# kronbichler/multigrid

Measured on AMD Instinct MI355X. Metric: DoFs/s for Laplace matvec + V-cycle, poisson_cube p=4 fp64, higher is better.
Workload: dtype f64; 1 GPU; poisson_cube FE_Q(4) 128^3 cells, 135005697 DoFs per GPU, 8 levels, step = 1 fp64 vmult + 1 V-cycle (Chebyshev degree 3, first kind); cells_per_dim=128, degree=4, n_dofs_per_gpu=135005697, global_dofs=135005697, parallelism=1 GPU

## Files before the change

### multigrid_amd/csrc/mgx_api.cpp

```cpp
#include "../../include/mgx.h"
#include "mgx_bricks.hpp"
#include "mgx_device_memory.hpp"
#include "mgx_internal.hpp"

#include <hip/hip_runtime.h>
#include <rccl/rccl.h>

#include <dlfcn.h>

#include <algorithm>
#include <chrono>
#include <cmath>
#include <cstdio>
#include <cstdlib>
#include <cstring>
#include <memory>
#include <string>
#include <type_traits>
#include <utility>
#include <vector>

using namespace mgx;

namespace
// ... 28 lines not shown
#ifndef MGX_CELLS_FORM
#define MGX_CELLS_FORM 0
#endif
extern "C" int mgx_has_cells_form(void) { return MGX_CELLS_FORM; }
extern "C" int64_t mgx_live_device_allocations(void) { return mgx::live_device_allocations().load(); }

mgx::Tunables mgx::Tunables::from_environment()
{
  Tunables t;
  auto     num = [](const char *name, uint32_t dflt) {
    const char *e = std::getenv(name);
    return e ? (uint32_t)std::strtoul(e, nullptr, 10) : dflt;
  };
  t.trace               = std::getenv("MGX_TRACE") != nullptr;
  t.brick_min           = num("MGX_BRICK_MIN", t.brick_min);
  t.brick_min_from_env  = std::getenv("MGX_BRICK_MIN") != nullptr;
  t.overlap_min         = num("MGX_OVERLAP_MIN_BRICKS", t.overlap_min);
  t.restrict_colour_min = num("MGX_RESTRICT_COLOUR_MIN", t.restrict_colour_min);
  t.cell_colour_min     = num("MGX_CELL_COLOUR_MIN", t.cell_colour_min);
  t.free_max_bricks     = num("MGX_FREE_MAX_BRICKS", t.free_max_bricks);
  t.free_one_max        = num("MGX_FREE_ONE_MAX", t.free_one_max);
  t.graph_max_dofs      = num("MGX_GRAPH_MAX_DOFS", t.graph_max_dofs);
  return t;
}

bool mgx::Tunables::set(const std::string &name, double value)
{
  const bool     on = value != 0.;
  const uint32_t u  = value <= 0. ? 0u : (value >= 4294967295. ? 0xFFFFFFFFu : (uint32_t)value);
  struct Entry
  {
    const char *name;
    bool       *flag;
    uint32_t   *number;
  };
  const Entry table[] = {
    {"trace", &trace, nullptr},
    {"brick_min", nullptr, &brick_min},
    {"overlap_min_bricks", nullptr, &overlap_min},
    {"restrict_colour_min", nullptr, &restrict_colour_min},
    {"cell_colour_min", nullptr, &cell_colour_min},
    {"free_max_bricks", nullptr, &free_max_bricks},
    {"free_one_max", nullptr, &free_one_max},
    {"graph_max_dofs", nullptr, &graph_max_dofs},
    {"general_kernel", &general_kernel, nullptr},
    {"no_bricks", &no_bricks, nullptr},
#if MGX_CELLS_FORM
    {"cells_form", &cells_form, nullptr},
    {"brick_wide_max", nullptr, &wide_max},
#endif
    {"macro_wg_per_cu_x16", nullptr, &macro_wg_x16},
    {"no_diag_table", &no_diag_table, nullptr},
    {"no_macro_v2", &no_macro_v2, nullptr},
    {"no_general_bricks", &no_general_bricks, nullptr},
    {"general_brick_min", nullptr, &general_brick_min},
    {"fused_prolong_min_bricks", nullptr, &fused_prolong_min_bricks},
    {"roctx", &roctx, nullptr},
    {"no_fused_init", &no_fused_init, nullptr},
    {"no_fused_restrict", &no_fused_restrict, nullptr},
    {"no_fused_prolong", &no_fused_prolong, nullptr},
    {"force_fused_transfers", &force_fused_transfers, nullptr},
    {"transfer_v1", &transfer_v1, nullptr},
    {"restrict_atomic", &restrict_atomic, nullptr},
    {"exchange_unfused", &exchange_unfused, nullptr},
    {"no_graph", &no_graph, nullptr},
    {"dg_no_overlap", &dg_no_overlap, nullptr},
    {"dg_unmerged_restrict", &dg_unmerged_restrict, nullptr},
    {"no_fused_decomposed", &no_fused_decomposed, nullptr},
    {"no_fused_assembly", &no_fused_assembly, nullptr},
    {"no_fused_residual", &no_fused_residual, nullptr},
    {"no_restrict_scratch", &no_restrict_scratch, nullptr},
    {"rccl_selftest", &rccl_selftest, nullptr},
  };
  for (const Entry &e : table)
    if (name == e.name)
      {
        if (e.flag)
          *e.flag = on;
        else
          *e.number = u;
        if (name == "brick_min")
          brick_min_from_env = true;
        return true;
      }
  return false;
}

struct ExchangePlan
{
  std::vector<uint32_t> not_owned_host;
  int                    plan_id = 0, number = MGX_F64, self_pos = 0;
  std::vector<int>       rank;
  std::vector<uint32_t>  count;
  std::vector<uint32_t *> index_dev;
  std::vector<void *>    send, recv;
  uint32_t              *shared_dev = nullptr, *not_owned_dev = nullptr;
  uint32_t               n_shared = 0, n_not_owned = 0;
  void                  *own_buf = nullptr;
  std::vector<uint32_t>  start;
  uint32_t              *all_index_dev = nullptr, *csr_start_dev = nullptr, *csr_pos_dev = nullptr;
  uint8_t               *all_seg_dev = nullptr, *csr_k_dev = nullptr;
  bool                   fused = false;
};

struct RcclApi
{
// ... 1452 lines not shown
                    ck[fill[j]++] = 255;
                if (k < e.n_neighbors)
                  for (uint32_t i = 0; i < e.count[k]; ++i)
                    {
                      const uint32_t j = slot[e.index[k][i]];
                      ck[fill[j]]   = (uint8_t)k;
                      cp[fill[j]++] = i;
                    }
              }
            MGX_TRY(op.mem.upload(&P->all_index_dev, all_index));
            MGX_TRY(op.mem.upload(&P->all_seg_dev, all_seg));
            MGX_TRY(op.mem.upload(&P->csr_start_dev, cs));
            MGX_TRY(op.mem.upload(&P->csr_k_dev, ck));
            MGX_TRY(op.mem.upload(&P->csr_pos_dev, cp));
            P->fused = true;
          }
      }
    ctx->plans.push_back({(size_t)desc->n_dofs, P.get()});
    op.plan = std::move(P);
    return MGX_OK;
  }
}

extern "C" {

int mgx_operator_create(mgx_context_t ctx, const mgx_operator_desc *desc, mgx_operator_t *out)
{
  MGX_TRY(validate_operator_desc(ctx, desc, out));
  std::unique_ptr<mgx_operator_s, int (*)(mgx_operator_t)> op(new mgx_operator_s, mgx_operator_destroy);
  op->ctx              = ctx;
  op->constrained_last = constrained_are_last(desc);
  const Tunables &tun  = ctx->tun;
  const int       p = desc->degree, n = p + 1;
  const size_t    n_entries = 27 * (size_t)desc->n_cells;
  OperatorData   &d  = op->d;
  d.p              = p;
  d.number         = desc->number;
  d.n_cells        = desc->n_cells;
  d.n_dofs         = desc->n_dofs;
  d.n_constrained  = desc->n_constrained;
  for (int i = 0; i < 6; ++i)
    d.coef[i] = desc->coef[i];
  std::memcpy(op->S, desc->shape_values, sizeof(double) * n * n);
  std::memcpy(op->D, desc->colloc_grad, sizeof(double) * n * n);
  std::memcpy(op->w, desc->qweights, sizeof(double) * n);
  d.full_tensor      = !desc->coef_q && (desc->coef[3] != 0. || desc->coef[4] != 0. || desc->coef[5] != 0.);
  const bool general = d.full_tensor || desc->coef_q;
  d.separable        = !tun.general_kernel && !general;
  d.cells_form       = tun.cells_form;
  d.wide_max         = tun.wide_max;
  d.macro_wg_x16     = tun.macro_wg_x16;
  d.n_cus            = context_cus(ctx);
  d.macro_v2         = !tun.no_macro_v2;
  MGX_HIP(hipSetDevice(ctx->device));
  MGX_TRY(op->mem.upload(&d.idx27, desc->idx27, n_entries));
  if (desc->idx27_plain)
    MGX_TRY(op->mem.upload(&d.idx27_plain, desc->idx27_plain, n_entries));
  MGX_TRY(op->mem.upload(&d.constrained, desc->constrained, desc->n_constrained, 1));
  MGX_TRY(upload_basis(*op));
  MGX_TRY(op->mem.alloc(&d.inv_diag, number_size(d.number) * d.n_dofs));
  if (general)
    MGX_TRY(upload_general_tables(*op, desc));
  if (general && (desc->n_cells >= tun.cell_colour_min || (size_t)n * n * n * desc->n_cells > kAssemblyMaxEntries))
    MGX_TRY(colour_cells(*op, desc));
  const bool macro_covers = d.separable && (uint64_t)desc->n_dofs * number_size(d.number) < 0xFFFFFFF0ull;
  if (!tun.no_bricks && !general && (MGX_CELLS_FORM ? (p <= 4 || d.separable) : macro_covers))
    MGX_TRY(build_brick_schedule(*op, desc, tun));
  if (general && p == 4 && !desc->exchange && !tun.no_bricks && !tun.no_general_bricks && desc->n_dofs < 0x3FFFFFFFu &&
      (uint64_t)desc->n_dofs * number_size(d.number) < 0xFFFFFFF0ull &&
      desc->n_cells / 64 >= tun.general_brick_min)
    MGX_TRY(build_general_brick_schedule(*op, desc));
  MGX_TRY(build_ordered_assembly(*op, desc));
  start_vector_statistics(*op, desc);
  if (desc->global_index)
    MGX_TRY(op->mem.upload(&op->global_index_dev, desc->global_index, desc->n_dofs));
  if (desc->exchange)
    MGX_TRY(build_exchange_plan(*op, desc, tun));
  *out = op.release();
  return MGX_OK;
}

int mgx_operator_exchange_buffers(mgx_operator_t op, int k, void **send, void **recv, uint32_t *count, int *rank)
{
  MGX_REQUIRE(op && op->plan && k >= 0 && k < (int)op->plan->rank.size(), "mgx_operator_exchange_buffers: bad argument");
  if (send)
    *send = op->plan->send[k];
  if (recv)
    *recv = op->plan->recv[k];
  if (count)
    *count = op->plan->count[k];
  if (rank)
    *rank = op->plan->rank[k];
  return MGX_OK;
}

int mgx_exchange_add(mgx_operator_t op, void *vec)
{
  MGX_REQUIRE(op && vec, "mgx_exchange_add: null argument");
  return exchange_add(op, vec);
}

int mgx_operator_destroy(mgx_operator_t op)
{
  if (!op)
    return MGX_OK;
  (void)hipStreamSynchronize(op->ctx->stream);
// ... 2230 lines not shown
```

### multigrid_amd/csrc/mgx_internal.hpp

```cpp
#pragma once

#include "../../include/mgx.h"

#include <hip/hip_runtime.h>

#include <algorithm>
#include <cstddef>
#include <cstdint>
#include <string>
#include <type_traits>
#include <vector>

struct mgx_context_s;

namespace mgx
{
  constexpr int      kMaxN    = MGX_MAX_DEGREE + 1;
  constexpr uint32_t kInvalid = 0xFFFFFFFFu;

  struct Tunables
  {
    bool     trace            = false;
    bool     general_kernel   = false;
    bool     no_bricks        = false;
    uint32_t brick_min        = 512;
    bool     brick_min_from_env = false;
    uint32_t overlap_min      = 16384;
    bool     cells_form       = false;
    uint32_t wide_max         = 1024;
    bool     dg_no_overlap    = false;
    bool     no_restrict_scratch = false;
    bool     no_fused_residual = false;
    bool     no_fused_assembly = false;
    bool     no_fused_decomposed = false;
    bool     dg_unmerged_restrict = false;
    uint32_t macro_wg_x16     = 0;
    bool     no_diag_table    = false;
    bool     roctx            = false;
    uint32_t fused_prolong_min_bricks = 8192;
    bool     no_general_bricks = false;
    uint32_t general_brick_min = 2048;
    bool     no_macro_v2      = false;
    bool     no_fused_init    = false;
    bool     no_fused_restrict = false;
    bool     no_fused_prolong = false;
    bool     force_fused_transfers = false;
    bool     transfer_v1      = false;
    bool     restrict_atomic  = false;
    uint32_t restrict_colour_min = 16384;
    bool     exchange_unfused = false;
    uint32_t cell_colour_min  = 0xFFFFFFFFu;
    uint32_t free_max_bricks  = 16384;
    uint32_t free_one_max     = 1024;
    bool     no_graph         = false;
    uint32_t graph_max_dofs   = 600000;
    bool     rccl_selftest    = false;
    static Tunables from_environment();
    bool            set(const std::string &name, double value);
  };

  template <typename T>
  struct EOMat
  {
    T ee[(kMaxN / 2) * (kMaxN / 2)];
    T eo[(kMaxN / 2) * (kMaxN / 2)];
    T mc[kMaxN / 2];
    T mhh;
  };

  template <typename T>
  struct Basis1D
  {
    T S[kMaxN * kMaxN];
    T D[kMaxN * kMaxN];
    T w[kMaxN];
    T P1[2 * kMaxN * kMaxN];
    EOMat<T> mass, lapl;
    T P1eo[2 * kMaxN * kMaxN];
  };

  struct FreeSchedule
  {
    int       n_classes = 0;
    int       n_groups = 0, n_iface_groups = 0;
    uint32_t  group_start[9] = {0};
    uint32_t *ent         = nullptr;
    uint32_t *surf_off    = nullptr;
    uint32_t  n_surf      = 0;
    void     *priv        = nullptr;
    uint32_t *surf_dof    = nullptr, *surf_start = nullptr, *surf_pos = nullptr;
    uint32_t  n_surf_dofs = 0, n_surf_shared = 0;
    bool      available() const { return ent != nullptr; }
  };

  struct BrickData
  {
    uint32_t  n_bricks  = 0;
    int       n_colours = 0;
    int       n_iface_groups = 0;
    uint32_t  colour_start[33] = {0};
    uint32_t *ent_base  = nullptr;
    uint8_t  *ent_flags = nullptr;
    uint32_t *item_map  = nullptr;
    uint32_t *item_map2 = nullptr;
    std::vector<uint32_t> order;
    uint32_t *order_dev = nullptr;
    bool      available() const { return n_bricks > 0; }
    FreeSchedule fr;
  };
  constexpr int kBrickEntities = 729;
  constexpr int kMaxColours    = 32;

  struct OperatorData
  {
    int       p        = 0;
    int       number   = 1;
    uint32_t  n_cells  = 0;
    uint32_t  n_dofs   = 0;
    uint32_t  n_constrained = 0;
    uint32_t *idx27         = nullptr;
    uint32_t *idx27_plain   = nullptr;
    uint32_t *constrained   = nullptr;
    void     *basis         = nullptr;
    void     *inv_diag      = nullptr;
    double    coef[6]       = {0, 0, 0, 0, 0, 0};
    bool      full_tensor   = false;
    void     *coef_q        = nullptr;
    void     *grad_1d       = nullptr;
    uint32_t *cell_order    = nullptr;
    int       n_cell_colours = 0;
    uint32_t  cell_colour_start[33] = {0};
    uint32_t *asm_start     = nullptr;
    uint32_t *asm_pos       = nullptr;
    void     *cell_scratch  = nullptr;
    BrickData bricks;
    BrickData gbricks;
    bool      cells_form    = false;
    uint32_t  wide_max      = 1024;
    uint32_t  macro_wg_x16  = 0;
    uint32_t  n_cus         = 256;
    bool      separable     = true;
    void     *diag_items    = nullptr;
    void     *diag_items2   = nullptr;
    bool      macro_v2      = true;
  };

  struct TransferData
  {
    const OperatorData *coarse = nullptr, *fine = nullptr;
    uint32_t           *children = nullptr;
    uint8_t            *weight_shift = nullptr;
    uint32_t           *own27 = nullptr;
    uint32_t           *patch = nullptr;
    uint32_t           *coarse_blocks = nullptr;
    void               *coarse_scratch = nullptr;
    uint32_t           *cs_start = nullptr, *cs_pos = nullptr;
    uint32_t           *ifr_cdof = nullptr, *ifr_start = nullptr, *ifr_fdof = nullptr;
    void               *ifr_w = nullptr;
    uint32_t            n_ifr = 0;
    uint32_t           *ifp_start = nullptr, *ifp_cdof = nullptr;
    void               *ifp_w = nullptr;
    uint32_t            n_ifp = 0;
    mutable uint32_t    pipe_grid[4] = {0, 0, 0, 0};
    bool                owner_weights = false;
    bool                coarse_coloured = false;
    uint32_t            n_cus = 256;
    uint32_t            colour_min = 16384;
  };

  int  exchange_buffers(struct ::mgx_context_s *ctx, int plan_id, int number, int n_neighbors, const int *ranks,
                        const uint32_t *counts, void *const *send, void *const *recv, hipStream_t stream = nullptr);
  hipStream_t side_stream_begin(struct ::mgx_context_s *ctx);
  int         side_stream_end(struct ::mgx_context_s *ctx);
  int  allreduce_sum(struct ::mgx_context_s *ctx, double *values, int count);
  int  dot_owned_prefix(struct ::mgx_context_s *ctx, int number, const void *x, const void *y, size_t n, double *out);
  bool context_has_comm(struct ::mgx_context_s *ctx);
  const Tunables &context_tunables(struct ::mgx_context_s *ctx);
  void tridiag_extreme_eigenvalues(int n, const double *d, const double *e, double &lo, double &hi);

  int report_error(int code, const char *message);
  inline int report_error(int code, const std::string &message) { return report_error(code, message.c_str()); }

#define MGX_HIP(call)                                                                                                \
  do                                                                                                                 \
    {                                                                                                                \
      hipError_t e_ = (call);                                                                                        \
      if (e_ != hipSuccess)                                                                                          \
        return mgx::report_error(MGX_ERR_HIP, std::string(#call) + ": " + hipGetErrorString(e_) + " (" + __FILE__ + ":" + \
                                                std::to_string(__LINE__) + ")");                                     \
    }                                                                                                                \
  while (0)

#define MGX_TRY(call)     \
  do                      \
    {                     \
      int s_ = (call);    \
      if (s_ != MGX_OK)   \
// ... 323 lines not shown
```

### multigrid_amd/csrc/mgx_macro.hip

```cpp
#include "mgx_macro_device.hpp"

#include <hip/hip_runtime.h>

#include <algorithm>
#include <cstdlib>

#ifndef MGX_MACRO_CHUNK
#define MGX_MACRO_CHUNK (MGX_MACRO_PAIRS ? 3 : 4)
#endif
#ifndef MGX_MACRO_CHUNK_CHEB
#define MGX_MACRO_CHUNK_CHEB (MGX_MACRO_PAIRS ? 2 : 3)
#endif
#ifndef MGX_MACRO_T
#define MGX_MACRO_T double
#endif

#ifdef MGX_MACRO_STAMPS
#ifndef MGX_MACRO_STAMP_MODE
#define MGX_MACRO_STAMP_MODE -1
#endif
__device__ unsigned long long g_mgx_stamps[8192 * 16];
#define MGX_STAMP(k)                                                                    \
  do                                                                                    \
    {                                                                                   \
      if (threadIdx.x == 0 && blockIdx.x < 8192 && (MGX_MACRO_STAMP_MODE < 0 || MODE == MGX_MACRO_STAMP_MODE)) \
        g_mgx_stamps[blockIdx.x * 16 + (k)] = ((k) == 15 || (k) == 13) ? __builtin_amdgcn_s_memrealtime() \
                                                        : __builtin_amdgcn_s_memtime();  \
    }                                                                                   \
  while (0)
extern "C" int mgx_debug_read_stamps(unsigned long long *host, int n_blocks)
{
  return (int)hipMemcpyFromSymbol(host, HIP_SYMBOL(g_mgx_stamps), sizeof(unsigned long long) * 16 * n_blocks);
}
#define MGX_STAMP_IT(k)      \
  do                         \
    {                        \
      if (mgx_iter == 3)     \
        MGX_STAMP(k);        \
    }                        \
  while (0)
#define MGX_STAMP_NEXT() ++mgx_iter
#define mgx_iter_is(k) (mgx_iter == (k))
#else
#define MGX_STAMP(k) ((void)0)
#define MGX_STAMP_IT(k) ((void)0)
#define MGX_STAMP_NEXT() ((void)0)
#define mgx_iter_is(k) false
#endif

namespace mgx
{
  template <int P, typename T, int MODE, bool DTAB, bool FREE = false>
  __global__ void __launch_bounds__((MCfg<P, T>::THREADS), (MCfg<P, T>::MINW))
    brick_macro_kernel(const T *__restrict__ src, uint32_t brick_first, uint32_t brick_count,
                       const uint32_t *__restrict__ ent_base, const uint32_t *__restrict__ item_map,
                       const Basis1D<T> *__restrict__ B, T c0, T c1, T c2, BrickPost<T> post, uint32_t vec_bytes)
  {
    using C              = MCfg<P, T>;
    constexpr int G      = C::G;
    constexpr int NT     = C::THREADS;
    constexpr int IT     = C::IT;
    constexpr int LINES  = C::LINES;
    constexpr int NEW    = (C::NE + NT - 1) / NT;
    constexpr int N = P + 1, NB = C::NB;
    constexpr int REM    = LINES - NT;
    constexpr bool kKeepX = is_cheb_mode(MODE) || MODE == kCgUpdate;
    constexpr int  NG     = ((MODE == kChebInit && !DTAB) || MODE == kCgUpdate) ? 2 : 1;
    __shared__ T U[C::ASZ];
    __shared__ T W[C::ASZ];

    const int tid = threadIdx.x;
    uint32_t  b   = blockIdx.x;
    if (b >= brick_count)
      return;
    MGX_STAMP(0);
    MGX_STAMP(15);
#ifdef MGX_MACRO_STAGGER
    if (__builtin_amdgcn_s_getreg(6 | (0 << 6) | ((8 - 1) << 11)) != 0)
      for (int i = 0; i < MGX_MACRO_STAGGER; ++i)
        __builtin_amdgcn_s_sleep(64);
#endif
    constexpr int NP = C::NPAIR, NS = C::NSINGLE, JP = C::JP, JS = C::JS, NU = JP + JS;
    auto live_p = [&](int j) { return (j + 1) * NT <= NP || tid + j * NT < NP; };
    auto live_s = [&](int j) { return (j + 1) * NT <= NS || tid + j * NT < NS; };
    auto live   = [&](int v) { return v < 2 * JP ? live_p(v / 2) : live_s(v - 2 * JP); };
    uint32_t mw[IT];
#pragma unroll
    for (int j = 0; j < JP; ++j)
      {
        const int     q = tid + j * NT;
        const u32x2_t m = reinterpret_cast<const u32x2_t *>(item_map)[q < NP ? q : 0];
        mw[2 * j]       = m.x;
        mw[2 * j + 1]   = m.y;
      }
#pragma unroll
    for (int j = 0; j < JS; ++j)
      {
        const int q    = tid + j * NT;
        mw[2 * JP + j] = item_map[2 * NP + (q < NS ? q : 0)];
      }
    T dv[DTAB ? IT : 1];
    if (DTAB)
      {
#pragma unroll
        for (int j = 0; j < JP; ++j)
// ... 41 lines not shown
#pragma unroll
      for (int j = 0; j < NEW; ++j)
        if (tid + j * NT < C::NE)
          E[tid + j * NT] = e[j];
    };
    auto unit_offset = [&](uint32_t w, uint32_t m, int it = 0, uint32_t brick = 0) {
#ifdef MGX_MACRO_CONTIG
      return w != kInvalid ? ((brick_first + brick) * (uint32_t)(C::NB * C::NB * C::NB * P * P * P) + (uint32_t)(tid + it * NT)) * (uint32_t)sizeof(T) : kOob;
#else
      return w != kInvalid ? (ent_index(w) + item_offset(m)) * (uint32_t)sizeof(T) : kOob;
#endif
    };
    constexpr bool kProlong = MODE == kChebFirstProlong;
    constexpr int  CNP = (C::NB / 2) * P + 1, NCV = CNP * CNP * CNP / NT + 1, CE3 = (C::NB + 1) * (C::NB + 1) * (C::NB + 1);
    T              cvv[NCV];
    T    g[NG][IT];
    uint32_t cw[NCV];
    auto coarse_words = [&](uint32_t brick) {
      if (kProlong)
        {
          const uint32_t *ctab = post.coarse_blocks + (size_t)(brick_first + brick) * CE3;
#pragma unroll
          for (int k = 0; k < NCV; ++k)
            {
              const int l = tid + k * NT;
              int       slot = 0, pnt;
              uint32_t  off;
              if (l < CNP * CNP * CNP)
                coarse_point<P>(l, slot, off, pnt);
              cw[k] = ctab[slot];
            }
        }
    };
    auto coarse_values = [&]() {
      if (kProlong)
        {
#pragma unroll
          for (int k = 0; k < NCV; ++k)
            {
              const int l = tid + k * NT;
              cvv[k]      = T(0);
              if (l < CNP * CNP * CNP)
                {
                  int      slot, pnt;
                  uint32_t off;
                  coarse_point<P>(l, slot, off, pnt);
                  const uint32_t w = cw[k];
                  const T        v = post.coarse[w != kInvalid ? w + off : 0u];
                  cvv[k]           = w != kInvalid ? v : T(0);
                }
            }
        }
    };
    auto gather_issue = [&](const uint32_t *E, uint32_t brick) {
      const rsrc_t r0 = MODE == kChebInit ? (DTAB ? R.a : R.b) : rsrc;
      const rsrc_t r1 = MODE == kCgUpdate ? R.b : R.a;
#pragma unroll
      for (int j = 0; j < JP; ++j)
        {
#pragma unroll
          for (int e = 0; e < 2; ++e)
            g[0][2 * j + e] = g[NG - 1][2 * j + e] = T(0);
          if (live_p(j))
            {
              const uint32_t off = unit_offset(E[item_slot(mw[2 * j])], mw[2 * j], 2 * j, brick);
              buf_ld2(r0, off, g[0][2 * j], g[0][2 * j + 1]);
              if (NG == 2)
                buf_ld2(r1, off, g[NG - 1][2 * j], g[NG - 1][2 * j + 1]);
            }
        }
#pragma unroll
      for (int j = 0; j < JS; ++j)
        {
          const int v = 2 * JP + j;
          g[0][v] = g[NG - 1][v] = T(0);
          if (live_s(j))
            {
              const uint32_t off = unit_offset(E[item_slot(mw[v])], mw[v], v, brick);
              g[0][v]            = buf_ld(r0, off, T());
              if (NG == 2)
                g[NG - 1][v] = buf_ld(r1, off, T());
            }
        }
    };
    T    xs[kKeepX ? IT : 1];
    auto gather_land = [&]() {
#pragma unroll
      for (int it = 0; it < IT; ++it)
        {
          T v = g[0][it];
          if (MODE == kChebInit)
            v = DTAB ? post.f0 * dv[DTAB ? it : 0] * g[0][it] : post.f0 * g[0][it] * g[NG - 1][it];
          if (MODE == kCgUpdate)
            v = post.f1 == T(0) ? g[NG - 1][it] : post.f2 * g[0][it] + g[NG - 1][it];
          if (live(it))
            U[item_point(mw[it])] = v;
          if (kKeepX)
            xs[it] = v;
        }
    };

    auto interpolate = [&]() {
      if (kProlong)
        {
          lds_barrier();
          prolong_brick<P, T, NT>(tid, W, B->P1eo, cvv);
        }
    };
    auto add_correction = [&]() {
      if (kProlong)
        {
#pragma unroll
          for (int it = 0; it < IT; ++it)
            if (live(it))
              {
                const uint32_t pnt = item_point(mw[it]);
                xs[kKeepX ? it : 0] += W[pnt];
                U[pnt] = xs[kKeepX ? it : 0];
              }
        }
    };

    table_load(b, ec);
    table_store(reinterpret_cast<uint32_t *>(W), ec);
    __syncthreads();
    MGX_STAMP(1);
    gather_issue(reinterpret_cast<const uint32_t *>(W), b);
    coarse_words(b);
    coarse_values();
    interpolate();
    gather_land();
// ... 137 lines not shown
            for (int i = 0; i < N; ++i)
              seg[i] = W[base + i * (G * G)];
            cell_apply<P, T>(K, seg, r);
#pragma unroll
            for (int i = 0; i < N; ++i)
              seg[i] = U[base + i * (G * G)];
            cell_apply<P, T>(M, seg, y);
#pragma unroll
            for (int i = 0; i < N; ++i)
              y[i] = fma(c2, r[i], y[i]);
            const T yn = next_lane(y[0]);
            if (c + 1 < NB)
              y[P] += yn;
#pragma unroll
            for (int i = 1; i < N; ++i)
              W[base + i * (G * G)] = y[i];
            if (c == 0)
              W[base] = y[0];
          }
        if (tid < LINES)
          {
            const int l = tid;
            T         a[G], r[G], o[G];
#pragma unroll
            for (int j = 0; j < G; ++j)
              a[j] = W[l + j * (G * G)];
            macro_apply<P, T>(K, a, r);
#pragma unroll
            for (int j = 0; j < G; ++j)
              a[j] = U[l + j * (G * G)];
            macro_apply<P, T>(M, a, o);
#pragma unroll
            for (int j = 0; j < G; ++j)
              W[l + j * (G * G)] = fma(c2, r[j], o[j]);
          }
          }
#endif
        __syncthreads();
        MGX_STAMP_IT(6);
        uint32_t *ebase = reinterpret_cast<uint32_t *>(U), *E2 = ebase + C::NE;
        table_store(ebase, ec);
        if (has_next)
          table_store(E2, en);
        const uint32_t *sbase = ebase + 2 * C::NE;
        if (FREE)
          {
#pragma unroll
            for (int j = 0; j < NEW; ++j)
              if (tid + j * NT < C::NE)
                ebase[2 * C::NE + tid + j * NT] = sc[FREE ? j : 0];
          }
        __syncthreads();
        constexpr bool kPipeGather = (MODE != kChebInit || DTAB) && MODE != kCgUpdate && MODE != kChebFirstProlong;
        if (has_next && kPipeGather)
          gather_issue(E2, bn);
        if (has_next)
          coarse_values();
        MGX_STAMP_IT(7);

        {
          constexpr int kChunk = MODE == kPlain ? NU : (MODE == kResidual ? (NU + 1) / 2 : (kKeepX ? MGX_MACRO_CHUNK_CHEB : MGX_MACRO_CHUNK)),
                        NCH    = (NU + kChunk - 1) / kChunk;
          PostOps<T>    ops[2][kChunk];
          uint32_t      iw[2][kChunk];
          uint32_t      pw[2][FREE ? kChunk : 1];
          const uint32_t priv0 = FREE ? (brick_first + b) * post.n_surf : 0u;
          auto slot0 = [&](int u) { return u < JP ? 2 * u : JP + u; };
          auto ulive = [&](int u) { return u < JP ? live_p(u) : live_s(u - JP); };
          auto issue = [&](int c, PostOps<T>(&o)[kChunk], uint32_t(&w)[kChunk], uint32_t(&pv)[FREE ? kChunk : 1]) {
#pragma unroll
            for (int j = 0; j < kChunk; ++j)
              {
                const int u = c * kChunk + j;
                w[j]        = kInvalid;
                if (u < NU && ulive(u))
                  w[j] = ebase[item_slot(mw[slot0(u)])];
                if (FREE)
                  {
                    const uint32_t so = (u < NU && ulive(u)) ? sbase[item_slot(mw[slot0(u < NU ? u : 0)])] : kInvalid;
                    const bool     vd = w[j] != kInvalid;
                    if (vd && so != kInvalid)
                      w[j] = ent_index(w[j]) | 0x40000000u;
                    pv[FREE ? j : 0] = (vd && so != kInvalid)
                                         ? (priv0 + so + item_offset(mw[slot0(u < NU ? u : 0)])) * (uint32_t)sizeof(T)
                                         : kOob;
                  }
              }
#pragma unroll
            for (int j = 0; j < kChunk; ++j)
              {
                const int u = c * kChunk + j;
                if (u < JP)
                  post_issue<T, MODE, DTAB, true>(R, w[j], unit_offset(w[j], mw[slot0(u < NU ? u : 0)], slot0(u < NU ? u : 0), b), o[j]);
                else if (u < NU)
                  post_issue<T, MODE, DTAB, false>(R, w[j], unit_offset(w[j], mw[slot0(u < NU ? u : 0)], slot0(u < NU ? u : 0), b), o[j]);
              }
          };
          issue(0, ops[0], iw[0], pw[0]);
#pragma unroll
          for (int c = 0; c < NCH; ++c)
            {
              if (c + 1 < NCH)
                issue(c + 1, ops[(c + 1) & 1], iw[(c + 1) & 1], pw[(c + 1) & 1]);
              __builtin_amdgcn_sched_barrier(0);
              T val[kChunk][2];
#pragma unroll
              for (int j = 0; j < kChunk; ++j)
                {
                  const int u = c * kChunk + j;
                  val[j][0] = val[j][1] = T(0);
                  if (u < NU && ulive(u))
                    {
                      val[j][0] = W[item_point(mw[slot0(u)])];
                      if (u < JP)
                        val[j][1] = W[item_point(mw[slot0(u) + 1])];
                    }
                }
#pragma unroll
              for (int j = 0; j < kChunk; ++j)
                {
                  const int u = c * kChunk + j;
                  if (u < NU)
                    {
                      const int         v0   = slot0(u);
                      const bool        pair = u < JP;
                      const uint32_t    w    = iw[c & 1][j];
                      const bool        vld  = w != kInvalid, last = vld && (w >> 31);
                      const uint32_t    off  = unit_offset(w, mw[v0], v0, b);
                      const PostOps<T> &o    = ops[c & 1][j];
                      T                 res[2];
#pragma unroll
                      for (int e = 0; e < 2; ++e)
                        res[e] = (e == 0 || pair)
                                   ? post_finish<T, MODE>(post, o.pv[e], o.av[e], o.ov[e], DTAB ? dv[DTAB ? v0 + e : 0] : o.bv[e],
                                                          last, val[j][e], xs[kKeepX ? v0 + e : 0])
                                   : T(0);
                      constexpr int kStAux = (MODE == kPlain || MODE == kResidual) ? kAuxNt : 0;
                      auto          st     = [&](rsrc_t r, uint32_t f) {
                        if (pair)
                          buf_st2(r, f, res[0], res[1]);
                        else
                          buf_st<kStAux>(r, f, res[0]);
                      };
                      if (MODE == kResidualRestrict)
                        {
                          if (ulive(u))
                            {
                              W[item_point(mw[v0])] = vld ? res[0] : T(0);
                              if (pair)
                                W[item_point(mw[v0 + 1])] = vld ? res[1] : T(0);
                            }
                        }
                      else if (MODE == kCgUpdate)
                        {
                          st(R.out, last ? off : kOob);
                          if (__builtin_amdgcn_ballot_w64(vld && !last) != 0)
                            st(R.partial, last ? kOob : off);
                          const T xn = o.ov[0] + post.f1 * o.bv[0];
                          buf_st(R.srcw, last ? off : kOob, xs[kKeepX ? v0 : 0]);
                          if (post.f1 != T(0))
                            buf_st(R.xw, last ? off : kOob, xn);
                          if (last)
                            {
                              const double qv = (double)res[0], pn = (double)xs[kKeepX ? v0 : 0], rv = (double)o.av[0];
                              cg[0] += qv * pn;
                              cg[1] += rv * rv;
                              cg[2] += qv * rv;
                              cg[3] += qv * qv;
                            }
                        }
                      else
                        {
                          st(R.out, last ? off : kOob);
                          if (FREE)
                            {
                              const uint32_t po = pw[c & 1][FREE ? j : 0];
                              if (__builtin_amdgcn_ballot_w64(po != kOob) != 0)
                                st(R.priv, po);
                              if (__builtin_amdgcn_ballot_w64(vld && !last && po == kOob) != 0)
                                st(R.partial, (last || po != kOob) ? kOob : off);
                            }
#ifndef MGX_MACRO_NOCARRIER
                          else if (__builtin_amdgcn_ballot_w64(vld && !last) != 0)
                            st(R.partial, last ? kOob : off);
#endif
                          if (MODE == kChebFirstProlong)
                            buf_st(R.srcw, last ? off : kOob, xs[kKeepX ? v0 : 0]);
                        }
                    }
                }
              __builtin_amdgcn_sched_barrier(0);
            }
        }
        MGX_STAMP_IT(8);
        if (MODE == kResidualRestrict)
          {
            constexpr int CE1 = C::NB + 1;
            __syncthreads();
            const uint32_t *ctab = post.coarse_blocks + (size_t)(brick_first + b) * (CE1 * CE1 * CE1);
            if (post.coarse_scratch)
              restrict_brick<P, T, NT, true>(tid, W, B->P1eo, nullptr, ctab,
                                             post.coarse_scratch + (size_t)(brick_first + b) * (CNP * CNP * CNP));
            else
              restrict_brick<P, T, NT, false>(tid, W, B->P1eo, post.coarse, ctab);
          }
        if (!has_next)
          break;
        if (!kPipeGather)
          gather_issue(E2, bn);
        __syncthreads();
#pragma unroll
        for (int j = 0; j < NEW; ++j)
          ec[j] = en[j];
        interpolate();
        gather_land();
        add_correction();
        MGX_STAMP_IT(9);
        __syncthreads();
        MGX_STAMP_IT(10);
        b = bn;
        MGX_STAMP_NEXT();
      }
    if (MODE == kCgUpdate)
      {
        static_assert(MODE != kCgUpdate || !MGX_MACRO_PAIRS, "kCgUpdate is written for single items");
        __syncthreads();
        double *red = reinterpret_cast<double *>(U);
#pragma unroll
        for (int k = 0; k < 4; ++k)
          red[k * NT + tid] = cg[k];
        __syncthreads();
        constexpr int P2 = NT <= 64 ? 64 : (NT <= 128 ? 128 : (NT <= 256 ? 256 : 512));
        for (int stride = P2 / 2; stride > 0; stride >>= 1)
          {
            if (tid < stride && tid + stride < NT)
              {
#pragma unroll
                for (int k = 0; k < 4; ++k)
                  red[k * NT + tid] += red[k * NT + tid + stride];
              }
            __syncthreads();
          }
        if (tid < 4)
          post.sums[blockIdx.x * 4 + tid] = red[tid * NT];
      }
#ifdef MGX_MACRO_STAMPS
    asm volatile("s_waitcnt vmcnt(0)" ::: "memory");
    MGX_STAMP(14);
    MGX_STAMP(13);
#endif
  }

  template <int P, typename T, int MODE, bool FREE>
  static void macro_launch(hipStream_t s, const OperatorData &op, const T *src, BrickPost<T> post, int g0, int g1)
  {
    using C                     = MCfg<P, T>;
    const BrickData &bd         = op.bricks;
    const uint32_t  *ent        = FREE ? bd.fr.ent : bd.ent_base;
    const uint32_t  *group_start = FREE ? bd.fr.group_start : bd.colour_start;
    if (FREE)
      {
        post.priv       = (T *)bd.fr.priv;
        post.surf_off   = bd.fr.surf_off;
        post.n_surf     = bd.fr.n_surf;
        post.priv_bytes = (uint32_t)((size_t)bd.n_bricks * bd.fr.n_surf * sizeof(T));
      }
    constexpr bool kUsesDiag = is_cheb_mode(MODE);
    const bool     dtab      = kUsesDiag && op.diag_items;
    if (dtab)
      post.b = (const T *)op.diag_items;
    const bool one_launch = MODE == kResidualRestrict && post.coarse_scratch != nullptr;
    for (int c = g0; c < g1; ++c)
      {
        uint32_t first = group_start[c], count = group_start[c + 1] - first;
        if (one_launch)
          {
            if (c != g0)
              break;
            count = group_start[g1] - first;
          }
        if (count == 0)
          continue;
        const uint32_t grid = persistent_grid(op, C::WGS, count);
        if (dtab)
          hipLaunchKernelGGL((brick_macro_kernel<P, T, MODE, kUsesDiag, FREE>), dim3(grid), dim3(C::THREADS), 0, s, src, first,
                             count, ent, bd.item_map, (const Basis1D<T> *)op.basis, (T)op.coef[0], (T)op.coef[1],
                             (T)op.coef[2], post, (uint32_t)(op.n_dofs * sizeof(T)));
        else
          hipLaunchKernelGGL((brick_macro_kernel<P, T, MODE, false, FREE>), dim3(grid), dim3(C::THREADS), 0, s, src, first,
                             count, ent, bd.item_map, (const Basis1D<T> *)op.basis, (T)op.coef[0], (T)op.coef[1],
                             (T)op.coef[2], post, (uint32_t)(op.n_dofs * sizeof(T)));
      }
  }

#if MGX_MACRO_IS_F64
  __global__ void reduce4_kernel(const double *__restrict__ partials, uint32_t n, const double *__restrict__ extra,
                                 double *__restrict__ sums)
  {
    __shared__ double red[4 * 256];
    const int         tid = threadIdx.x;
    double            acc[4] = {0., 0., 0., 0.};
    for (uint32_t i = tid; i < n; i += 256)
      for (int k = 0; k < 4; ++k)
        acc[k] += partials[4 * (size_t)i + k];
    for (int k = 0; k < 4; ++k)
      red[k * 256 + tid] = acc[k];
    __syncthreads();
    for (int stride = 128; stride > 0; stride >>= 1)
      {
        if (tid < stride)
          for (int k = 0; k < 4; ++k)
            red[k * 256 + tid] += red[k * 256 + tid + stride];
        __syncthreads();
      }
    if (tid < 4)
      sums[tid] = red[tid * 256] + (extra ? extra[tid] : 0.);
  }
#endif

  template <typename T, bool VERIFY>
  __global__ void diag_table_kernel(const T *__restrict__ inv_diag, const uint32_t *__restrict__ ent_base,
                                    const uint32_t *__restrict__ item_map, uint32_t ne, uint32_t npts, T *table,
                                    uint32_t *flag)
  {
    const uint32_t brick = blockIdx.x;
    for (uint32_t i = threadIdx.x; i < npts; i += blockDim.x)
      {
        const uint32_t m = item_map[i], w = ent_base[(size_t)brick * ne + item_slot(m)];
        if (w == kInvalid)
          continue;
        const T v = inv_diag[ent_index(w) + item_offset(m)];
        if (!VERIFY)
          table[i] = v;
        else
          {
            const T    t   = table[i];
            const T    tol = (sizeof(T) == 8 ? T(1e-14) : T(2e-6)) * (t < 0 ? -t : t);
            const T    dvt = v - t;
            const bool same = (dvt < 0 ? -dvt : dvt) <= tol;
            if (!same)
              atomicOr(flag, 1u);
          }
      }
  }
// ... 101 lines not shown
```

### multigrid_amd/csrc/mgx_macro2.hip

```cpp
#include "mgx_macro_device.hpp"

#include <hip/hip_runtime.h>

#include <algorithm>
#include <cstdlib>

#ifndef MGX_MACRO_T
#define MGX_MACRO_T double
#endif
#ifndef MGX_MACRO2_CHUNK
#define MGX_MACRO2_CHUNK 3
#endif

#ifdef MGX_MACRO_STAMPS
#ifndef MGX_MACRO_STAMP_MODE
#define MGX_MACRO_STAMP_MODE -1
#endif
__device__ unsigned long long g_mgx_stamps2[8192 * 16];
#define MGX_STAMP(k)                                                                                              \
  do                                                                                                              \
    {                                                                                                             \
      if (threadIdx.x == 0 && blockIdx.x < 8192 && (MGX_MACRO_STAMP_MODE < 0 || MODE == MGX_MACRO_STAMP_MODE))      \
        g_mgx_stamps2[blockIdx.x * 16 + (k)] = ((k) == 15 || (k) == 13) ? __builtin_amdgcn_s_memrealtime()         \
                                                                         : __builtin_amdgcn_s_memtime();           \
// ... 146 lines not shown
#pragma unroll
        for (int j = 0; j < G; ++j)
          U[base + j * G] = fma(c0, t2[j], c1 * s2[j]);
      }
    lds_barrier();
    mark(1);
    if (REM > 0 && tid < REM * NB)
      {
        const int l = NT + tid / NB, c = tid % NB, base = l + c * P * (G * G);
        T         seg[N], y[N], r[N];
#pragma unroll
        for (int i = 0; i < N; ++i)
          seg[i] = W[base + i * (G * G)];
        cell_apply<P, T>(K, seg, r);
#pragma unroll
        for (int i = 0; i < N; ++i)
          seg[i] = U[base + i * (G * G)];
        cell_apply<P, T>(M, seg, y);
#pragma unroll
        for (int i = 0; i < N; ++i)
          y[i] = fma(c2, r[i], y[i]);
        const T yn = next_lane(y[0]);
        if (c + 1 < NB)
          y[P] += yn;
#pragma unroll
        for (int i = 1; i < N; ++i)
          W[base + i * (G * G)] = y[i];
        if (c == 0)
          W[base] = y[0];
      }
    if (tid < LINES)
      {
        const int l = tid;
        T         a[G], r[G], o[G];
#pragma unroll
        for (int j = 0; j < G; ++j)
          a[j] = W[l + j * (G * G)];
        macro_apply<P, T>(K, a, r);
#pragma unroll
        for (int j = 0; j < G; ++j)
          a[j] = U[l + j * (G * G)];
        macro_apply<P, T>(M, a, o);
#pragma unroll
        for (int j = 0; j < G; ++j)
          W[l + j * (G * G)] = fma(c2, r[j], o[j]);
      }
  }

  __host__ __device__ constexpr bool macro2_covers(int mode, int p)
  {
    return mode == kPlain || mode == kResidual || ((mode == kResidualRestrict || mode == kChebInit) && p <= 4) || mode == kChebOldInit;
  }

  template <int P, typename T, int MODE>
  __global__ void __launch_bounds__((M2Cfg<P, T>::THREADS), (M2Cfg<P, T>::MINW))
    brick_macro2_kernel(const T *__restrict__ src, uint32_t brick_first, uint32_t brick_count,
                        const uint32_t *__restrict__ ent_base, const uint32_t *__restrict__ item_map,
                        const Basis1D<T> *__restrict__ B, T c0, T c1, T c2, BrickPost<T> post, uint32_t vec_bytes)
  {
    static_assert(macro2_covers(MODE, P), "form not covered by this pipeline");
    using C            = M2Cfg<P, T>;
    constexpr int NT   = C::THREADS, IT = C::IT, JINT = C::JINT, JSURF = C::JSURF, NE = C::NE;
    constexpr int NEW  = (NE + NT - 1) / NT;
    __shared__ T        U[C::ASZ];
    __shared__ T        W[C::ASZ];
    __shared__ uint32_t E[NE];

    const int tid = threadIdx.x;
    uint32_t  b   = blockIdx.x;
    if (b >= brick_count)
      return;
    MGX_STAMP(0);
    MGX_STAMP(15);
#ifdef MGX_MACRO_STAMPS
    int mgx_iter = 0;
#endif
    auto live = [&](int j) { return (j + 1) * NT <= C::NPTS || tid + j * NT < C::NPTS; };
    uint32_t mw[IT];
#pragma unroll
    for (int j = 0; j < IT; ++j)
      mw[j] = item_map[live(j) ? tid + j * NT : 0];
    const rsrc_t rsrc = make_rsrc(src, vec_bytes), r_a = make_rsrc(post.a, vec_bytes), r_out = make_rsrc(post.out, vec_bytes),
                 r_partial = make_rsrc(post.partial, vec_bytes), r_old = make_rsrc(post.old, vec_bytes);
    const EOMat<T> &M = B->mass, &K = B->lapl;
    constexpr bool kKeepX = is_cheb_mode(MODE);
    T              dv[kKeepX ? IT : 1];
    if (kKeepX)
      {
#pragma unroll
        for (int j = 0; j < IT; ++j)
          dv[kKeepX ? j : 0] = post.b[live(j) ? tid + j * NT : 0];
      }

    uint32_t en[NEW] = {};
    auto     table_load = [&](uint32_t brick, uint32_t(&e)[NEW]) {
#pragma unroll
      for (int j = 0; j < NEW; ++j)
        {
          const int i = tid + j * NT;
          e[j]        = ent_base[(size_t)(brick_first + brick) * NE + (i < NE ? i : 0)];
        }
    };
    auto table_store = [&](uint32_t *dst, const uint32_t(&e)[NEW]) {
#pragma unroll
      for (int j = 0; j < NEW; ++j)
        if (tid + j * NT < NE)
          dst[tid + j * NT] = e[j];
    };
    auto unit_offset = [&](uint32_t w, uint32_t m) {
      return w != kInvalid ? (ent_index(w) + item_offset(m)) * (uint32_t)sizeof(T) : kOob;
    };
    T    g[IT];
    auto gather_issue = [&](const uint32_t *tab) {
#pragma unroll
      for (int j = 0; j < IT; ++j)
        {
          g[j] = T(0);
          if (live(j))
            g[j] = buf_ld(MODE == kChebInit ? r_a : rsrc, unit_offset(tab[item_slot(mw[j])], mw[j]), T());
        }
    };
    T    xs[kKeepX ? IT : 1];
    auto gather_land = [&]() {
#pragma unroll
      for (int j = 0; j < IT; ++j)
        {
          T v = g[j];
          if (MODE == kChebInit)
            v = post.f0 * dv[kKeepX ? j : 0] * g[j];
          if (live(j))
            U[item_point(mw[j])] = v;
          if (kKeepX)
            xs[kKeepX ? j : 0] = v;
        }
    };
    constexpr bool kCarrier = MODE != kResidualRestrict;
    T              pp[JSURF];
    auto           partial_issue = [&]() {
#pragma unroll
      for (int j = JINT; j < IT; ++j)
        {
          pp[j - JINT] = T(0);
          if (!kCarrier)
            continue;
#ifndef MGX_MACRO_NOCARRIER
          const uint32_t w    = live(j) ? E[item_slot(mw[j])] : kInvalid;
          const bool     need = w != kInvalid && !(w & 0x40000000u);
          if (__builtin_amdgcn_ballot_w64(need) != 0)
            pp[j - JINT] = buf_ld(r_partial, need ? unit_offset(w, mw[j]) : kOob, T());
#endif
        }
    };

    constexpr bool kRhs = MODE == kResidual || MODE == kResidualRestrict;
    T              av[kRhs ? IT : 1];
    auto           rhs_issue = [&]() {
      if (kRhs)
        {
#pragma unroll
          for (int j = 0; j < IT; ++j)
            {
              const uint32_t w    = live(j) ? E[item_slot(mw[j])] : kInvalid;
              const bool     last = w != kInvalid && (j < JINT || (w >> 31));
              av[kRhs ? j : 0]    = buf_ld(r_a, last ? unit_offset(w, mw[j]) : kOob, T());
            }
        }
    };

    {
      uint32_t e0[NEW];
      table_load(b, e0);
      if (b + gridDim.x < brick_count)
        table_load(b + gridDim.x, en);
      table_store(E, e0);
      lds_barrier();
      MGX_STAMP(1);
      gather_issue(E);
      gather_land();
      MGX_STAMP(2);
      lds_barrier();
    }

    for (;;)
      {
        const uint32_t bn = b + gridDim.x;
        const bool     has_next = bn < brick_count;
        MGX_STAMP_IT(3);
#ifdef MGX_MACRO_STAMPS
        if (mgx_iter == 4)
          MGX_STAMP(11);
#endif
        partial_issue();
        rhs_issue();
#pragma unroll
        for (int j = 0; j < IT; ++j)
          asm volatile("" : "+v"(mw[j]));
        if (MODE == kChebInit || MODE == kChebOldInit)
          {
#pragma unroll
            for (int j = 0; j < IT; ++j)
              asm volatile("" : "+v"(dv[kKeepX ? j : 0]));
          }
        MGX_STAMP_IT(4);
#ifndef MGX_MACRO_NOSWEEP
        if (kSlicedSweeps<P, MODE> && P >= 9)
          brick_sweeps_sliced<P, T>(
            tid, U, W, B, c0, c1, c2, [&](int k) { MGX_STAMP_IT(5 + k); }, [&]() { lds_barrier(); });
        else
          brick_sweeps<P, T>(tid, U, W, M, K, c0, c1, c2, [&](int k) { MGX_STAMP_IT(5 + k); });
#endif
        lds_barrier();
        MGX_STAMP_IT(7);
        if (has_next)
          {
            table_store(reinterpret_cast<uint32_t *>(U), en);
            lds_barrier();
            gather_issue(reinterpret_cast<const uint32_t *>(U));
          }
        MGX_STAMP_IT(8);

        if constexpr (kKeepX)
          {
            constexpr int kChunk = MGX_MACRO2_CHUNK < IT ? MGX_MACRO2_CHUNK : IT, NCH = (IT + kChunk - 1) / kChunk;
            struct Ops
            {
              T        av, ov;
              uint32_t w, off;
            };
            Ops  ops[2][kChunk];
            auto issue = [&](int c, Ops(&o)[kChunk]) {
#pragma unroll
              for (int k = 0; k < kChunk; ++k)
                {
                  const int j = c * kChunk + k;
                  if (j < IT)
                    o[k].w = live(j) ? E[item_slot(mw[j])] : kInvalid;
                }
#pragma unroll
              for (int k = 0; k < kChunk; ++k)
                {
                  const int j = c * kChunk + k;
                  if (j >= IT)
                    continue;
                  if (j < JINT && o[k].w != kInvalid)
                    o[k].w |= 0xC0000000u;
                  const bool last  = o[k].w != kInvalid && (o[k].w >> 31);
                  o[k].off         = unit_offset(o[k].w, mw[j]);
                  const uint32_t ol = last ? o[k].off : kOob;
                  o[k].av          = buf_ld(r_a, ol, T());
                  o[k].ov          = MODE == kCheb ? buf_ld(r_old, ol, T()) : T(0);
                }
            };
            issue(0, ops[0]);
#pragma unroll
            for (int c = 0; c < NCH; ++c)
              {
                if (c + 1 < NCH)
                  issue(c + 1, ops[(c + 1) & 1]);
                __builtin_amdgcn_sched_barrier(0);
                T val[kChunk];
#pragma unroll
                for (int k = 0; k < kChunk; ++k)
                  {
                    const int j = c * kChunk + k;
                    val[k]      = (j < IT && live(j)) ? W[item_point(mw[j])] : T(0);
                  }
#pragma unroll
                for (int k = 0; k < kChunk; ++k)
                  {
                    const int j = c * kChunk + k;
                    if (j >= IT)
                      continue;
                    const Ops &o   = ops[c & 1][k];
                    const bool vld = o.w != kInvalid, last = vld && (o.w >> 31);
                    const T    res = post_finish<T, MODE>(post, j >= JINT ? pp[j >= JINT ? j - JINT : 0] : T(0), o.av, o.ov,
                                                          dv[kKeepX ? j : 0], last, val[k], xs[kKeepX ? j : 0]);
                    if (j < JINT)
                      buf_st(r_out, o.off, res);
                    else
                      {
                        buf_st(r_out, last ? o.off : kOob, res);
#ifndef MGX_MACRO_NOCARRIER
                        if (__builtin_amdgcn_ballot_w64(vld && !last) != 0)
                          buf_st(r_partial, last ? kOob : o.off, res);
#endif
                      }
                  }
                __builtin_amdgcn_sched_barrier(0);
              }
          }
        else
          {
          {
            uint32_t w[IT];
  #pragma unroll
            for (int j = 0; j < IT; ++j)
              w[j] = live(j) ? E[item_slot(mw[j])] : kInvalid;
  #pragma unroll
            for (int j = 0; j < IT; ++j)
              {
                if (j < JINT && w[j] != kInvalid)
                  w[j] |= 0xC0000000u;
                const bool     vld = w[j] != kInvalid, last = vld && (w[j] >> 31);
                const uint32_t off = unit_offset(w[j], mw[j]);
                T              val = live(j) ? W[item_point(mw[j])] : T(0);
                if (j >= JINT && kCarrier)
                  val += pp[j >= JINT ? j - JINT : 0];
                if (MODE == kResidualRestrict)
                  {
                    if (live(j))
                      W[item_point(mw[j])] = vld ? (last ? av[kRhs ? j : 0] : T(0)) - val : T(0);
                    continue;
                  }
                if (MODE == kResidual && last)
                  val = av[kRhs ? j : 0] - val;
                if (j < JINT)
                  buf_st<kAuxNt>(r_out, off, val);
                else
                  {
                    buf_st<kAuxNt>(r_out, last ? off : kOob, val);
  #ifndef MGX_MACRO_NOCARRIER
                    if (__builtin_amdgcn_ballot_w64(vld && !last) != 0)
                      buf_st(r_partial, last ? kOob : off, val);
  #endif
                  }
              }
          }
          }
        if (MODE == kResidualRestrict)
          {
            constexpr int CE1 = C::NB + 1, CNP = (C::NB / 2) * P + 1;
            lds_barrier();
            const uint32_t *ctab = post.coarse_blocks + (size_t)(brick_first + b) * (CE1 * CE1 * CE1);
            if (post.coarse_scratch)
              restrict_brick<P, T, NT, true>(tid, W, B->P1eo, nullptr, ctab,
                                             post.coarse_scratch + (size_t)(brick_first + b) * (CNP * CNP * CNP));
            else
              restrict_brick<P, T, NT, false>(tid, W, B->P1eo, post.coarse, ctab);
          }
        MGX_STAMP_IT(9);
        if (!has_next)
          break;
        lds_barrier();
        gather_land();
        table_store(E, en);
        if (bn + gridDim.x < brick_count)
          table_load(bn + gridDim.x, en);
        MGX_STAMP_IT(10);
        lds_barrier();
        b = bn;
#ifdef MGX_MACRO_STAMPS
        ++mgx_iter;
#endif
      }
#ifdef MGX_MACRO_STAMPS
    asm volatile("s_waitcnt vmcnt(0)" ::: "memory");
    MGX_STAMP(14);
    MGX_STAMP(13);
#endif
  }

  template <int P, typename T, int MODE>
  static void macro2_launch(hipStream_t s, const OperatorData &op, const T *src, const BrickPost<T> &post, int g0, int g1)
  {
    using C             = M2Cfg<P, T>;
    const BrickData &bd = op.bricks;
    const bool one_launch = MODE == kResidualRestrict && post.coarse_scratch != nullptr;
    for (int c = g0; c < g1; ++c)
      {
        uint32_t first = bd.colour_start[c], count = bd.colour_start[c + 1] - first;
        if (one_launch)
          {
            if (c != g0)
              break;
            count = bd.colour_start[g1] - first;
          }
        if (count == 0)
          continue;
        const uint32_t grid = persistent_grid(op, C::WGS, count);
        hipLaunchKernelGGL((brick_macro2_kernel<P, T, MODE>), dim3(grid), dim3(C::THREADS), 0, s, src, first, count, bd.ent_base,
                           bd.item_map2, (const Basis1D<T> *)op.basis, (T)op.coef[0], (T)op.coef[1], (T)op.coef[2], post,
                           (uint32_t)(op.n_dofs * sizeof(T)));
      }
  }

#define MGX_CAT2(a, b) a##b
#define MGX_CAT(a, b) MGX_CAT2(a, b)
  bool MGX_CAT(launch_macro2_loop_, MGX_MACRO_SUFFIX)(hipStream_t s, const OperatorData &op, const BrickLaunch &l)
  {
    using T = MGX_MACRO_T;
    if (!macro2_covers(l.mode, op.p) || !op.bricks.item_map2 || (uint64_t)op.n_dofs * sizeof(T) >= 0xFFFFFFF0ull)
      return false;
    if (is_cheb_mode(l.mode) && !op.diag_items2)
      return false;
    BrickPost<T> post = make_post<T>(l);
    post.b            = (const T *)op.diag_items2;
    bool launched     = false;
    dispatch_degree(op.p, [&](auto degree) {
      constexpr int P = decltype(degree)::value;
      dispatch_mode<kPlain, kResidual, kChebInit, kChebOldInit, kResidualRestrict>(l.mode, [&](auto form) {
        constexpr int MODE = decltype(form)::value;
        if constexpr (macro2_covers(MODE, P))
          {
            macro2_launch<P, T, MODE>(s, op, (const T *)l.src, post, l.group_begin, l.group_end);
            launched = true;
          }
      });
    });
    return launched;
  }
}
```

Measured before the change: 14.93 billion DoFs/s.

## Stream next-brick gather loads chunk by chunk inside Chebyshev macro kernels

```diff
diff --git a/multigrid_amd/csrc/mgx_api.cpp b/multigrid_amd/csrc/mgx_api.cpp
--- a/multigrid_amd/csrc/mgx_api.cpp
+++ b/multigrid_amd/csrc/mgx_api.cpp
@@ -104,6 +104,7 @@
     {"macro_wg_per_cu_x16", nullptr, &macro_wg_x16},
     {"no_diag_table", &no_diag_table, nullptr},
     {"no_macro_v2", &no_macro_v2, nullptr},
+    {"no_streamed_gather", &no_streamed_gather, nullptr},
     {"no_general_bricks", &no_general_bricks, nullptr},
     {"general_brick_min", nullptr, &general_brick_min},
     {"fused_prolong_min_bricks", nullptr, &fused_prolong_min_bricks},
@@ -1662,6 +1663,7 @@
   d.macro_wg_x16     = tun.macro_wg_x16;
   d.n_cus            = context_cus(ctx);
   d.macro_v2         = !tun.no_macro_v2;
+  d.streamed_gather  = !tun.no_streamed_gather;
   MGX_HIP(hipSetDevice(ctx->device));
   MGX_TRY(op->mem.upload(&d.idx27, desc->idx27, n_entries));
   if (desc->idx27_plain)
diff --git a/multigrid_amd/csrc/mgx_internal.hpp b/multigrid_amd/csrc/mgx_internal.hpp
--- a/multigrid_amd/csrc/mgx_internal.hpp
+++ b/multigrid_amd/csrc/mgx_internal.hpp
@@ -41,6 +41,7 @@
     bool     no_general_bricks = false;
     uint32_t general_brick_min = 2048;
     bool     no_macro_v2      = false;
+    bool     no_streamed_gather = false;
     bool     no_fused_init    = false;
     bool     no_fused_restrict = false;
     bool     no_fused_prolong = false;
@@ -143,6 +144,7 @@
     void     *diag_items    = nullptr;
     void     *diag_items2   = nullptr;
     bool      macro_v2      = true;
+    bool      streamed_gather = true;
   };
 
   struct TransferData
diff --git a/multigrid_amd/csrc/mgx_macro.hip b/multigrid_amd/csrc/mgx_macro.hip
--- a/multigrid_amd/csrc/mgx_macro.hip
+++ b/multigrid_amd/csrc/mgx_macro.hip
@@ -50,7 +50,13 @@
 
 namespace mgx
 {
-  template <int P, typename T, int MODE, bool DTAB, bool FREE = false>
+  __host__ __device__ constexpr bool macro_streams(int mode, bool dtab, int p, bool reduced_colours, bool fp32)
+  {
+    return fp32 && is_cheb_mode(mode) && (mode != kChebInit || dtab) && (mode != kChebFirstProlong || p <= 4) &&
+           !(mode == kCheb && dtab && p == 3 && reduced_colours);
+  }
+
+  template <int P, typename T, int MODE, bool DTAB, bool FREE = false, bool STREAM = false>
   __global__ void __launch_bounds__((MCfg<P, T>::THREADS), (MCfg<P, T>::MINW))
     brick_macro_kernel(const T *__restrict__ src, uint32_t brick_first, uint32_t brick_count,
                        const uint32_t *__restrict__ ent_base, const uint32_t *__restrict__ item_map,
@@ -198,31 +204,31 @@
             }
         }
     };
-    auto gather_issue = [&](const uint32_t *E, uint32_t brick) {
+    auto gather_issue = [&](const uint32_t *E, uint32_t brick, int u0 = 0, int u1 = C::JP + C::JS, bool next = true) {
       const rsrc_t r0 = MODE == kChebInit ? (DTAB ? R.a : R.b) : rsrc;
       const rsrc_t r1 = MODE == kCgUpdate ? R.b : R.a;
 #pragma unroll
-      for (int j = 0; j < JP; ++j)
+      for (int j = u0; j < (u1 < JP ? u1 : JP); ++j)
         {
 #pragma unroll
           for (int e = 0; e < 2; ++e)
             g[0][2 * j + e] = g[NG - 1][2 * j + e] = T(0);
-          if (live_p(j))
+          if (STREAM || live_p(j))
             {
-              const uint32_t off = unit_offset(E[item_slot(mw[2 * j])], mw[2 * j], 2 * j, brick);
+              const uint32_t off = (!STREAM || (next && live_p(j))) ? unit_offset(E[item_slot(mw[2 * j])], mw[2 * j], 2 * j, brick) : kOob;
               buf_ld2(r0, off, g[0][2 * j], g[0][2 * j + 1]);
               if (NG == 2)
                 buf_ld2(r1, off, g[NG - 1][2 * j], g[NG - 1][2 * j + 1]);
             }
         }
 #pragma unroll
-      for (int j = 0; j < JS; ++j)
+      for (int j = (u0 > JP ? u0 - JP : 0); j < (u1 - JP < JS ? u1 - JP : JS); ++j)
         {
           const int v = 2 * JP + j;
           g[0][v] = g[NG - 1][v] = T(0);
-          if (live_s(j))
+          if (STREAM || live_s(j))
             {
-              const uint32_t off = unit_offset(E[item_slot(mw[v])], mw[v], v, brick);
+              const uint32_t off = (!STREAM || (next && live_s(j))) ? unit_offset(E[item_slot(mw[v])], mw[v], v, brick) : kOob;
               g[0][v]            = buf_ld(r0, off, T());
               if (NG == 2)
                 g[NG - 1][v] = buf_ld(r1, off, T());
@@ -466,7 +472,8 @@
           }
         __syncthreads();
         constexpr bool kPipeGather = (MODE != kChebInit || DTAB) && MODE != kCgUpdate && MODE != kChebFirstProlong;
-        if (has_next && kPipeGather)
+        static_assert(!STREAM || macro_streams(MODE, DTAB, P, FREE, sizeof(T) == 4), "this form does not stream its gather");
+        if (has_next && kPipeGather && !STREAM)
           gather_issue(E2, bn);
         if (has_next)
           coarse_values();
@@ -516,7 +523,17 @@
             {
               if (c + 1 < NCH)
                 issue(c + 1, ops[(c + 1) & 1], iw[(c + 1) & 1], pw[(c + 1) & 1]);
+              if (STREAM)
+                gather_issue(E2, bn, c * kChunk, (c + 1) * kChunk, has_next);
               __builtin_amdgcn_sched_barrier(0);
+#ifdef MGX_MACRO_STAMPS
+              if (c == 0)
+                {
+                  const PostOps<T> &o = ops[0][(NU < kChunk ? NU : kChunk) - 1];
+                  asm volatile("" ::"v"(o.pv[0]), "v"(o.av[0]), "v"(o.bv[0]), "v"(o.ov[0]));
+                  MGX_STAMP_IT(12);
+                }
+#endif
               T val[kChunk][2];
 #pragma unroll
               for (int j = 0; j < kChunk; ++j)
@@ -620,7 +637,7 @@
           }
         if (!has_next)
           break;
-        if (!kPipeGather)
+        if (!kPipeGather && !STREAM)
           gather_issue(E2, bn);
         __syncthreads();
 #pragma unroll
@@ -696,14 +713,20 @@
         if (count == 0)
           continue;
         const uint32_t grid = persistent_grid(op, C::WGS, count);
-        if (dtab)
-          hipLaunchKernelGGL((brick_macro_kernel<P, T, MODE, kUsesDiag, FREE>), dim3(grid), dim3(C::THREADS), 0, s, src, first,
-                             count, ent, bd.item_map, (const Basis1D<T> *)op.basis, (T)op.coef[0], (T)op.coef[1],
-                             (T)op.coef[2], post, (uint32_t)(op.n_dofs * sizeof(T)));
+        auto launch = [&](auto dt, auto st) {
+          hipLaunchKernelGGL((brick_macro_kernel<P, T, MODE, decltype(dt)::value, FREE, decltype(st)::value>), dim3(grid),
+                             dim3(C::THREADS), 0, s, src, first, count, ent, bd.item_map, (const Basis1D<T> *)op.basis,
+                             (T)op.coef[0], (T)op.coef[1], (T)op.coef[2], post, (uint32_t)(op.n_dofs * sizeof(T)));
+        };
+        using std::bool_constant;
+        if (dtab && op.streamed_gather)
+          launch(bool_constant<kUsesDiag>(), bool_constant<macro_streams(MODE, kUsesDiag, P, FREE, sizeof(T) == 4)>());
+        else if (dtab)
+          launch(bool_constant<kUsesDiag>(), bool_constant<false>());
+        else if (op.streamed_gather)
+          launch(bool_constant<false>(), bool_constant<macro_streams(MODE, false, P, FREE, sizeof(T) == 4)>());
         else
-          hipLaunchKernelGGL((brick_macro_kernel<P, T, MODE, false, FREE>), dim3(grid), dim3(C::THREADS), 0, s, src, first,
-                             count, ent, bd.item_map, (const Basis1D<T> *)op.basis, (T)op.coef[0], (T)op.coef[1],
-                             (T)op.coef[2], post, (uint32_t)(op.n_dofs * sizeof(T)));
+          launch(bool_constant<false>(), bool_constant<false>());
       }
   }
 
diff --git a/multigrid_amd/csrc/mgx_macro2.hip b/multigrid_amd/csrc/mgx_macro2.hip
--- a/multigrid_amd/csrc/mgx_macro2.hip
+++ b/multigrid_amd/csrc/mgx_macro2.hip
@@ -222,13 +222,14 @@
     return mode == kPlain || mode == kResidual || ((mode == kResidualRestrict || mode == kChebInit) && p <= 4) || mode == kChebOldInit;
   }
 
-  template <int P, typename T, int MODE>
+  template <int P, typename T, int MODE, bool STREAM = false>
   __global__ void __launch_bounds__((M2Cfg<P, T>::THREADS), (M2Cfg<P, T>::MINW))
     brick_macro2_kernel(const T *__restrict__ src, uint32_t brick_first, uint32_t brick_count,
                         const uint32_t *__restrict__ ent_base, const uint32_t *__restrict__ item_map,
                         const Basis1D<T> *__restrict__ B, T c0, T c1, T c2, BrickPost<T> post, uint32_t vec_bytes)
   {
     static_assert(macro2_covers(MODE, P), "form not covered by this pipeline");
+    static_assert(!STREAM || is_cheb_mode(MODE), "only the Chebyshev forms stream the gather");
     using C            = M2Cfg<P, T>;
     constexpr int NT   = C::THREADS, IT = C::IT, JINT = C::JINT, JSURF = C::JSURF, NE = C::NE;
     constexpr int NEW  = (NE + NT - 1) / NT;
@@ -281,13 +282,16 @@
       return w != kInvalid ? (ent_index(w) + item_offset(m)) * (uint32_t)sizeof(T) : kOob;
     };
     T    g[IT];
-    auto gather_issue = [&](const uint32_t *tab) {
-#pragma unroll
-      for (int j = 0; j < IT; ++j)
+    auto gather_issue = [&](const uint32_t *tab, int j0 = 0, int j1 = C::IT, bool next = true) {
+      const rsrc_t r0 = MODE == kChebInit ? r_a : rsrc;
+#pragma unroll
+      for (int j = j0; j < (j1 < IT ? j1 : IT); ++j)
         {
           g[j] = T(0);
-          if (live(j))
-            g[j] = buf_ld(MODE == kChebInit ? r_a : rsrc, unit_offset(tab[item_slot(mw[j])], mw[j]), T());
+          if (STREAM)
+            g[j] = buf_ld(r0, (next && live(j)) ? unit_offset(tab[item_slot(mw[j])], mw[j]) : kOob, T());
+          else if (live(j))
+            g[j] = buf_ld(r0, unit_offset(tab[item_slot(mw[j])], mw[j]), T());
         }
     };
     T    xs[kKeepX ? IT : 1];
@@ -385,7 +389,8 @@
           {
             table_store(reinterpret_cast<uint32_t *>(U), en);
             lds_barrier();
-            gather_issue(reinterpret_cast<const uint32_t *>(U));
+            if (!STREAM)
+              gather_issue(reinterpret_cast<const uint32_t *>(U));
           }
         MGX_STAMP_IT(8);
 
@@ -427,7 +432,16 @@
               {
                 if (c + 1 < NCH)
                   issue(c + 1, ops[(c + 1) & 1]);
+                if (STREAM)
+                  gather_issue(reinterpret_cast<const uint32_t *>(U), c * kChunk, (c + 1) * kChunk, has_next);
                 __builtin_amdgcn_sched_barrier(0);
+#ifdef MGX_MACRO_STAMPS
+                if (c == 0)
+                  {
+                    asm volatile("" ::"v"(ops[0][kChunk - 1].av), "v"(ops[0][kChunk - 1].ov));
+                    MGX_STAMP_IT(12);
+                  }
+#endif
                 T val[kChunk];
 #pragma unroll
                 for (int k = 0; k < kChunk; ++k)
@@ -530,7 +544,7 @@
 #endif
   }
 
-  template <int P, typename T, int MODE>
+  template <int P, typename T, int MODE, bool STREAM = false>
   static void macro2_launch(hipStream_t s, const OperatorData &op, const T *src, const BrickPost<T> &post, int g0, int g1)
   {
     using C             = M2Cfg<P, T>;
@@ -548,7 +562,7 @@
         if (count == 0)
           continue;
         const uint32_t grid = persistent_grid(op, C::WGS, count);
-        hipLaunchKernelGGL((brick_macro2_kernel<P, T, MODE>), dim3(grid), dim3(C::THREADS), 0, s, src, first, count, bd.ent_base,
+        hipLaunchKernelGGL((brick_macro2_kernel<P, T, MODE, STREAM>), dim3(grid), dim3(C::THREADS), 0, s, src, first, count, bd.ent_base,
                            bd.item_map2, (const Basis1D<T> *)op.basis, (T)op.coef[0], (T)op.coef[1], (T)op.coef[2], post,
                            (uint32_t)(op.n_dofs * sizeof(T)));
       }
@@ -572,7 +586,10 @@
         constexpr int MODE = decltype(form)::value;
         if constexpr (macro2_covers(MODE, P))
           {
-            macro2_launch<P, T, MODE>(s, op, (const T *)l.src, post, l.group_begin, l.group_end);
+            if (is_cheb_mode(MODE) && op.streamed_gather)
+              macro2_launch<P, T, MODE, is_cheb_mode(MODE)>(s, op, (const T *)l.src, post, l.group_begin, l.group_end);
+            else
+              macro2_launch<P, T, MODE>(s, op, (const T *)l.src, post, l.group_begin, l.group_end);
             launched = true;
           }
       });
```

Result: slower. 14.58 billion DoFs/s (-2.4%).
